# icyveins7/pydsproutines

Measured on AMD Instinct MI355X. Metric: CAF Msamples/s (4k template x 256 freq bins), higher is better.
Workload: dtype f32

## Files before the change

### pydsproutines_amd/csrc/caf_fft_dev.h

```cpp
#pragma once
#ifndef __HIPCC_RTC__
#include <hip/hip_runtime.h>
#endif

namespace caf {

__device__ __forceinline__ float2 cadd(float2 a, float2 b) { return make_float2(a.x + b.x, a.y + b.y); }
__device__ __forceinline__ float2 csub(float2 a, float2 b) { return make_float2(a.x - b.x, a.y - b.y); }
__device__ __forceinline__ float2 cmul(float2 a, float2 b) {
    return make_float2(__builtin_fmaf(a.x, b.x, -(a.y * b.y)), __builtin_fmaf(a.x, b.y, a.y * b.x));
}
__device__ __forceinline__ float2 mulj(float2 a) { return make_float2(-a.y, a.x); }
__device__ __forceinline__ void idft4(float2& a0, float2& a1, float2& a2, float2& a3) {
    const float2 s02 = cadd(a0, a2), d02 = csub(a0, a2);
    const float2 s13 = cadd(a1, a3), d13 = mulj(csub(a1, a3));
    a0 = cadd(s02, s13);
    a1 = cadd(d02, d13);
    a2 = csub(s02, s13);
    a3 = csub(d02, d13);
}

__device__ __forceinline__ void idft16(float2 (&v)[16]) {
    constexpr float C1 = 0.92387953251128674f;
    constexpr float S1 = 0.38268343236508977f;
    constexpr float R2 = 0.70710678118654752f;
#pragma unroll
    for (int m2 = 0; m2 < 4; ++m2) idft4(v[m2], v[4 + m2], v[8 + m2], v[12 + m2]);
    {
        const float2 w1 = make_float2(C1, S1), w3 = make_float2(S1, C1);
        v[4 * 1 + 1] = cmul(v[4 * 1 + 1], w1);
        v[4 * 2 + 1] = make_float2((v[4 * 2 + 1].x - v[4 * 2 + 1].y) * R2, (v[4 * 2 + 1].x + v[4 * 2 + 1].y) * R2);
        v[4 * 3 + 1] = cmul(v[4 * 3 + 1], w3);
        v[4 * 1 + 2] = make_float2((v[4 * 1 + 2].x - v[4 * 1 + 2].y) * R2, (v[4 * 1 + 2].x + v[4 * 1 + 2].y) * R2);
        v[4 * 2 + 2] = mulj(v[4 * 2 + 2]);
        v[4 * 3 + 2] = make_float2((-v[4 * 3 + 2].x - v[4 * 3 + 2].y) * R2, (v[4 * 3 + 2].x - v[4 * 3 + 2].y) * R2);
        v[4 * 1 + 3] = cmul(v[4 * 1 + 3], w3);
        v[4 * 2 + 3] = make_float2((-v[4 * 2 + 3].x - v[4 * 2 + 3].y) * R2, (v[4 * 2 + 3].x - v[4 * 2 + 3].y) * R2);
        v[4 * 3 + 3] = cmul(v[4 * 3 + 3], make_float2(-C1, -S1));
    }
#pragma unroll
    for (int n1 = 0; n1 < 4; ++n1) idft4(v[4 * n1 + 0], v[4 * n1 + 1], v[4 * n1 + 2], v[4 * n1 + 3]);
#pragma unroll
    for (int a = 0; a < 4; ++a)
#pragma unroll
        for (int b = a + 1; b < 4; ++b) {
            const float2 t = v[4 * a + b];
            v[4 * a + b] = v[4 * b + a];
            v[4 * b + a] = t;
        }
}

__device__ __forceinline__ void idft2(float2& a0, float2& a1) {
    const float2 s = cadd(a0, a1), d = csub(a0, a1);
    a0 = s;
    a1 = d;
}
__device__ __forceinline__ void idft8(float2 (&v)[8]) {
    constexpr float R2 = 0.70710678118654752f;
    float2 e0 = v[0], e1 = v[2], e2 = v[4], e3 = v[6];
    float2 o0 = v[1], o1 = v[3], o2 = v[5], o3 = v[7];
    idft4(e0, e1, e2, e3);
    idft4(o0, o1, o2, o3);
    o1 = make_float2((o1.x - o1.y) * R2, (o1.x + o1.y) * R2);
    o2 = mulj(o2);
    o3 = make_float2((-o3.x - o3.y) * R2, (o3.x - o3.y) * R2);
    v[0] = cadd(e0, o0);
    v[4] = csub(e0, o0);
    v[1] = cadd(e1, o1);
    v[5] = csub(e1, o1);
    v[2] = cadd(e2, o2);
    v[6] = csub(e2, o2);
    v[3] = cadd(e3, o3);
    v[7] = csub(e3, o3);
}

__device__ __forceinline__ void idft3(float2& x0, float2& x1, float2& x2) {
    constexpr float S = 0.86602540378443865f;
    const float2 t = cadd(x1, x2), d = csub(x1, x2);
    const float2 a = make_float2(x0.x - 0.5f * t.x, x0.y - 0.5f * t.y);
    const float2 b = make_float2(S * d.x, S * d.y);
    x0 = cadd(x0, t);
    x1 = make_float2(a.x - b.y, a.y + b.x);
    x2 = make_float2(a.x + b.y, a.y - b.x);
}
__device__ __forceinline__ void idft5(float2& x0, float2& x1, float2& x2, float2& x3, float2& x4) {
    constexpr float C1 = 0.30901699437494742f, C2 = -0.80901699437494742f;
    constexpr float S1 = 0.95105651629515357f, S2 = 0.58778525229247313f;
    const float2 t1 = cadd(x1, x4), t2 = cadd(x2, x3), t3 = csub(x1, x4), t4 = csub(x2, x3);
    const float2 a1 = make_float2(x0.x + C1 * t1.x + C2 * t2.x, x0.y + C1 * t1.y + C2 * t2.y);
    const float2 a2 = make_float2(x0.x + C2 * t1.x + C1 * t2.x, x0.y + C2 * t1.y + C1 * t2.y);
    const float2 b1 = make_float2(S1 * t3.x + S2 * t4.x, S1 * t3.y + S2 * t4.y);
    const float2 b2 = make_float2(S2 * t3.x - S1 * t4.x, S2 * t3.y - S1 * t4.y);
    x0 = make_float2(x0.x + t1.x + t2.x, x0.y + t1.y + t2.y);
    x1 = make_float2(a1.x - b1.y, a1.y + b1.x);
    x4 = make_float2(a1.x + b1.y, a1.y - b1.x);
    x2 = make_float2(a2.x - b2.y, a2.y + b2.x);
    x3 = make_float2(a2.x + b2.y, a2.y - b2.x);
}
__device__ __forceinline__ void idft10(float2 (&v)[10]) {
    float2 e0 = v[0], e1 = v[2], e2 = v[4], e3 = v[6], e4 = v[8];
    float2 o0 = v[1], o1 = v[3], o2 = v[5], o3 = v[7], o4 = v[9];
    idft5(e0, e1, e2, e3, e4);
    idft5(o0, o1, o2, o3, o4);
    o1 = cmul(o1, make_float2(0.80901699437494742f, 0.58778525229247313f));
    o2 = cmul(o2, make_float2(0.30901699437494742f, 0.95105651629515357f));
    o3 = cmul(o3, make_float2(-0.30901699437494742f, 0.95105651629515357f));
    o4 = cmul(o4, make_float2(-0.80901699437494742f, 0.58778525229247313f));
    v[0] = cadd(e0, o0), v[5] = csub(e0, o0);
    v[1] = cadd(e1, o1), v[6] = csub(e1, o1);
    v[2] = cadd(e2, o2), v[7] = csub(e2, o2);
    v[3] = cadd(e3, o3), v[8] = csub(e3, o3);
    v[4] = cadd(e4, o4), v[9] = csub(e4, o4);
}
__device__ __forceinline__ uint32_t fp_m2(uint32_t tid) {
    const uint32_t lane = tid & 63, wave = tid >> 6;
    const uint32_t b = (lane & 3) + 4 * (wave & 3), c = ((lane >> 2) & 3) + 4 * (wave >> 2), d = lane >> 4;
    return 64 * b + 4 * c + d;
}
__host__ __device__ __forceinline__ uint32_t fp_tid_of(uint32_t m2) {
    const uint32_t b = m2 >> 6, c = (m2 >> 2) & 15, d = m2 & 3;
    return (b & 3) | ((c & 3) << 2) | (d << 4) | ((b >> 2) << 6) | ((c >> 2) << 8);
}

}
```

### pydsproutines_amd/csrc/caf_fused.hip

```cpp
#include <algorithm>
#include <cstdlib>
#include <type_traits>

#include "caf_internal.h"
#include "caf_fft_dev.h"
#include "caf_wave.h"

namespace caf {

constexpr int FB = 16384;
constexpr int FP_P1 = 4384;
constexpr int FP_IM = 16 * FP_P1;
constexpr int F_LDS_BYTES = 2 * FP_IM;
constexpr int F_LDS_DATA = F_LDS_BYTES / 8;
__host__ __device__ constexpr int fp_row2(int n2) { return ((n2 >> 1) & 3) * 1088 + ((n2 & 1) + 2 * (n2 >> 3)) * 256; }
static_assert(fp_row2(15) + 256 <= FP_P1 && FP_P1 % 256 == 32, "planar image geometry");

#define CAF_AS1 __attribute__((address_space(1)))
#define CAF_AS4 __attribute__((address_space(4)))
typedef float v2f_t __attribute__((ext_vector_type(2)));
typedef float v4f_t __attribute__((ext_vector_type(4)));
typedef int v2i_t __attribute__((ext_vector_type(2)));
__device__ __forceinline__ float2 ld2(const float2* base, uint32_t elem) {
    const uint64_t u = *reinterpret_cast<const CAF_AS1 uint64_t*>((const CAF_AS1 char*)base + (elem << 3));
// ... 69 lines not shown
__device__ __forceinline__ float2 tw_ld(lds_tw_ptr b, int k) {
    const uint64_t u = b[k];
    float2 r;
    __builtin_memcpy(&r, &u, 8);
    return r;
}
__device__ __forceinline__ uint32_t fp_hbase(uint32_t m2, int32_t shift) {
    const uint32_t t = m2 - (uint32_t)shift;
    return (t & ~1023u) + fp_tid_of(t & 1023u);
}
__device__ __forceinline__ uint32_t fp_rd2(uint32_t tid) {
    const uint32_t lane = tid & 63, wave = tid >> 6;
    return wave * FP_P1 + (lane >> 4) * 1024 + (lane & 15) * 16;
}
__device__ __forceinline__ uint32_t fp_cd2(uint32_t tid) {
    const uint32_t lane = tid & 63;
    return 4 * ((lane & 3) + 4 * (lane >> 4)) + ((lane >> 2) & 3);
}
__device__ __forceinline__ uint32_t fp_rd3(uint32_t tid) {
    const uint32_t lane = tid & 63, wave = tid >> 6, n2 = lane >> 2;
    return wave * FP_P1 + ((n2 >> 1) & 3) * 1088 + ((n2 & 1) + 2 * (n2 >> 3)) * 256 + (lane & 3) * 16;
}
__device__ __forceinline__ uint32_t fp_rd4(uint32_t tid) {
    return (tid & 15) * FP_P1 + (tid >> 8) * 256 + ((tid >> 4) & 15) * 16;
}

template <typename Tp>
__device__ __forceinline__ Tp* uniform_ptr(Tp* p) {
    const uint64_t v = reinterpret_cast<uint64_t>(p);
    const uint32_t lo = __builtin_amdgcn_readfirstlane((uint32_t)v);
    const uint32_t hi = __builtin_amdgcn_readfirstlane((uint32_t)(v >> 32));
    return reinterpret_cast<Tp*>(((uint64_t)hi << 32) | lo);
}
__device__ __forceinline__ __amdgpu_buffer_rsrc_t buf_of(const void* base, uint32_t bytes) {
    return __builtin_amdgcn_make_buffer_rsrc(const_cast<void*>(base), 0, (int)bytes, 0x00020000);
}
constexpr int CAF_AUX_SC1 = 16;
constexpr int CAF_AUX_NT = 2;
template <int MODE>
__device__ __forceinline__ void tile_store(__amdgpu_buffer_rsrc_t r, uint32_t voff, uint32_t soff, float val) {
    __builtin_amdgcn_raw_buffer_store_b32(__builtin_bit_cast(int, val), r, (int)voff, (int)soff, MODE == 1 ? (CAF_AUX_SC1 | CAF_AUX_NT) : 0);
}

struct F1Direct {
    float* out0;
    float* out1;
    const float* inv_e;
    const float* tscale;
    int64_t num_shifts;
    int32_t step, blk_abs;
    PeakRec* partial;
    int64_t ppt, shift_start;
};
template <int FT, int MODE = 0, int NV4 = 4, bool PK = false>
__device__ __forceinline__ void fused_item(float2* __restrict__ s_d, const float2* __restrict__ s_tw2,
                                           const float2* __restrict__ s_tw3,
                                           const float2* __restrict__ xb,
                                           const float2* __restrict__ hc,
                                           const int32_t* __restrict__ shifts,
                                           const float2* __restrict__ tw1,
                                           int32_t table_mode, int32_t nfreq, int32_t nhyp, int blk, int h0, int h1,
                                           int32_t tiles_per_blk, float* __restrict__ vt,
                                           int32_t* __restrict__ imax = nullptr, const F1Direct* f1 = nullptr) {
    static_assert(FT == 1024, "one radix-16 butterfly per thread and pass: 1024 threads (wave w owns plane n1 = w)");
    constexpr int BPT = 1;
    const int tid = threadIdx.x;
    const lds_char* img = (const lds_char*)s_d;
    const uint32_t img0 = __builtin_amdgcn_readfirstlane((uint32_t)(uintptr_t)img);
    const uint32_t wave_u = __builtin_amdgcn_readfirstlane((uint32_t)tid >> 6);
    const uint32_t m0_x1 = img0 + wave_u * 256u, m0_w = img0 + wave_u * (uint32_t)FP_P1;
    const uint32_t m2 = fp_m2((uint32_t)tid);
    constexpr int nv4 = NV4;
    float bv[16];
    uint32_t bi[4];
    float ge[16];
    if (MODE == 2 || MODE == 5) {
#pragma unroll
        for (int o = 0; o < 16; ++o) bv[o] = -1.f;
#pragma unroll
        for (int o = 0; o < 4; ++o) bi[o] = 0u;
    }
    uint32_t f1_bytes = 0;
    int64_t f1_rel0 = 0;
    if (MODE >= 3) {
        f1_rel0 = (int64_t)f1->blk_abs * f1->step;
        int64_t nv = f1->num_shifts - f1_rel0;
        if (nv > f1->step) nv = f1->step;
        f1_bytes = (uint32_t)nv * 4u;
        const __amdgpu_buffer_rsrc_t rie = buf_of(uniform_ptr(f1->inv_e + f1_rel0), f1_bytes);
        const int n1 = tid & 15, n2 = (tid >> 4) & 15, q = tid >> 8;
#pragma unroll
        for (int i = 0; i < 4; ++i)
#pragma unroll
            for (int n4 = 0; n4 < 4; ++n4)
                ge[4 * i + n4] = __builtin_bit_cast(
                    float, __builtin_amdgcn_raw_buffer_load_b32(rie, (((n2 >> 2) + 4 * q) * 64 + n1 + 16 * (n2 & 3)) * 4,
                                                                (16 * i + 64 * n4) * 256, 0));
        if (MODE == 4) {
#pragma unroll
            for (int o = 0; o < 16; ++o) ge[o] = __builtin_sqrtf(ge[o]);
        }
    }

    uint32_t pk_d0 = 0, pk_nv = 0;
    if (PK) {
        const int n1 = tid & 15, n2 = (tid >> 4) & 15, q = tid >> 8;
        pk_d0 = (uint32_t)(((n2 >> 2) + 4 * q) * 64 + n1 + 16 * (n2 & 3));
        pk_nv = f1_bytes >> 2;
    }
    float2 w[BPT];
    const float2* xp = xb + (int64_t)blk * FB;
#pragma unroll
    for (int j = 0; j < BPT; ++j) w[j] = ld2(tw1, 1024u + m2);
    float* vt_blk = vt + (int64_t)blk * tiles_per_blk * nhyp * 64;
    const __amdgpu_buffer_rsrc_t rvt = buf_of(uniform_ptr(vt_blk), (uint32_t)tiles_per_blk * (uint32_t)nhyp * 256u);

    const float2* hrow_cur;
    uint32_t hb_cur;
    auto row_of = [&](int h) {
        if (table_mode) {
            hrow_cur = hc + (int64_t)h * FB;
            hb_cur = (uint32_t)tid;
        } else {
            const int t = h / nfreq;
            const int32_t sh = *((const CAF_AS4 int32_t*)shifts + (h - t * nfreq));
// ... 48 lines not shown
            float2 p = w[j];
            asm volatile("" : "+v"(p.x), "+v"(p.y));
            const float2 wj = p;
            v1[j][1] = cmul(v1[j][1], p);
#pragma unroll
            for (int n1 = 2; n1 < 16; ++n1) {
                p = cmul(p, wj);
                v1[j][n1] = cmul(v1[j][n1], p);
            }
        }
        __syncthreads();
        lds_rows16c<FP_P1>(m0_x1, v1[0]);
        __syncthreads();
        row_of(more ? h + 1 : h);
        constexpr int EH = MODE == 5 ? 2 : MODE >= 2 ? 5 : 0;
        float2 he[2 * EH + 1];
        constexpr int HP2 = 5;
        float2 hn[BPT][16];
        if (MODE < 2) {
#pragma unroll
            for (int a = 0; a < HP2; ++a) hn[0][a] = ld2(hrow_cur, ((1024u * a + hb_cur) & (FB - 1)) + lz);
        }
#pragma unroll
        for (int a = 0; a < EH; ++a) he[a] = ld2(hrow_cur, ((1024u * a + hb_cur) & (FB - 1)) + lz);
        {
            float2 v[16];
            const uint32_t rd2 = fp_rd2((uint32_t)(tid + lz)), rd2i = fp_im(rd2);
            const lds_tw_ptr t2 = tw_base(s_tw2, fp_cd2((uint32_t)(tid + lz)));
#pragma unroll
            for (int bh = 0; bh < 4; ++bh) lds_get4c(img, rd2 + 256u * bh, rd2i + 256u * bh, v[4 * bh], v[4 * bh + 1], v[4 * bh + 2], v[4 * bh + 3]);
            idft16(v);
#pragma unroll
            for (int n2 = 1; n2 < 16; ++n2) v[n2] = cmul(v[n2], tw_ld(t2, n2 * 64));
            lds_rows16c_x2(m0_w, v);
        }
#pragma unroll
        for (int a = 0; a < EH; ++a) pr[0][a] = cmul(xr[0][a], he[a]);
        __builtin_amdgcn_wave_barrier();
        if (MODE < 2) {
#pragma unroll
            for (int j = 0; j < BPT; ++j)
#pragma unroll
                for (int a = HP2; a < 16; ++a)
                    hn[j][a] = ld2(hrow_cur, (1024u * a + hb_cur) & (FB - 1));
        }
#pragma unroll
        for (int a = EH; a < 2 * EH; ++a) he[a] = ld2(hrow_cur, ((1024u * a + hb_cur) & (FB - 1)) + lz);
        {
            float2 v[16];
            const uint32_t rd3 = fp_rd3((uint32_t)(tid + lz)), rd3i = fp_im(rd3);
#pragma unroll
            for (int ch = 0; ch < 4; ++ch) lds_get4c(img, rd3 + 64u * ch, rd3i + 64u * ch, v[4 * ch], v[4 * ch + 1], v[4 * ch + 2], v[4 * ch + 3]);
            idft16(v);
            const lds_tw_ptr t3 = tw_base(s_tw3, (uint32_t)((tid & 3) + lz));
#pragma unroll
            for (int n3 = 1; n3 < 16; ++n3) v[n3] = cmul(v[n3], tw_ld(t3, n3 * 4));
            lds_rows16c<256>(m0_w, v);
        }
#pragma unroll
        for (int a = EH; a < 2 * EH; ++a) pr[0][a] = cmul(xr[0][a], he[a]);
        if (MODE >= 2) {
#pragma unroll
            for (int j = 0; j < BPT; ++j)
#pragma unroll
                for (int a = 2 * EH; a < 16; ++a)
                    hn[j][a] = ld2(hrow_cur, (1024u * a + hb_cur) & (FB - 1));
        }
        __syncthreads();
#pragma unroll
        for (int j = 0; j < BPT; ++j) {
            const int idx = tid + j * FT;
            const int n1 = idx & 15, n2 = (idx >> 4) & 15, q = idx >> 8;
            const uint32_t rd4 = fp_rd4((uint32_t)idx), rd4i = fp_im(rd4);
            __builtin_amdgcn_sched_barrier(0);
            float2 pf0, pf1, pf2, pf3;
            if (MODE < 2) {
                lds_get4c(img, rd4, rd4i, pf0, pf1, pf2, pf3);
                __builtin_amdgcn_sched_barrier(0);
#pragma unroll
                for (int a = 0; a < 16; ++a) pr[j][a] = cmul(xr[j][a], hn[j][a]);
                __builtin_amdgcn_sched_barrier(0);
            }
#pragma unroll
            for (int i = 0; i < 4; ++i) {
                uint32_t lzi = 0;
                asm volatile("" : "+v"(lzi));
                float2 a0, a1, a2, a3;
                if (MODE < 2 && i == 0)
                    a0 = pf0, a1 = pf1, a2 = pf2, a3 = pf3;
                else
                    lds_get4c(img, rd4 + 1024u * i + lzi, rd4i + 1024u * i + lzi, a0, a1, a2, a3);
                const float2 s02 = cadd(a0, a2), d02 = csub(a0, a2), s13 = cadd(a1, a3), d13 = mulj(csub(a1, a3));
#pragma unroll
                for (int n4 = 0; n4 < 4; ++n4) {
                    if (n4 >= nv4) continue;
                    const float2 yq = n4 == 0 ? cadd(s02, s13) : n4 == 1 ? cadd(d02, d13) : n4 == 2 ? csub(s02, s13) : csub(d02, d13);
                    const int tile_u = 16 * i + 64 * n4;
                    const int tile_t = (n2 >> 2) + 4 * q;
                    const uint32_t soff = (uint32_t)tile_u * (uint32_t)nhyp * 256u + hoff;
                    const uint32_t voff = ((uint32_t)tile_t * (uint32_t)nhyp * 64u + (uint32_t)(n1 + 16 * (n2 & 3))) << 2;
                    const float val = __builtin_fmaf(yq.x, yq.x, yq.y * yq.y);
                    if (MODE == 2) {
                        constexpr int o = 0;
                        (void)o;
                        const int oo = 4 * i + n4;
                        const bool up = val > bv[oo];
                        bv[oo] = up ? val : bv[oo];
                        const uint32_t sh8 = 8u * (uint32_t)(oo & 3);
                        const uint32_t repl = (bi[oo >> 2] & ~(0xffu << sh8)) | ((uint32_t)(h - h0) << sh8);
                        bi[oo >> 2] = up ? repl : bi[oo >> 2];
                    } else if (MODE == 5) {
                        const int oo = 4 * i + n4;
                        const float outv = val * (ge[oo] * f1_ts);
                        const bool up = outv > bv[oo];
                        bv[oo] = up ? outv : bv[oo];
                        const uint32_t sh8 = 8u * (uint32_t)(oo & 3);
                        const uint32_t repl = (bi[oo >> 2] & ~(0xffu << sh8)) | ((uint32_t)(h - h0) << sh8);
                        bi[oo >> 2] = up ? repl : bi[oo >> 2];
                        const uint32_t v3 = (uint32_t)(tile_t * 64 + n1 + 16 * (n2 & 3)) << 2, s3 = (uint32_t)tile_u * 256u;
                        __builtin_amdgcn_raw_buffer_store_b32(__builtin_bit_cast(int, outv), f1_r0, (int)v3, (int)s3, CAF_AUX_NT);
                    } else if (MODE == 4) {
                        const float gq = ge[4 * i + n4] * f1_ts;
                        const v2f_t ov = {yq.x * gq, yq.y * gq};
                        const uint32_t v3 = (uint32_t)(tile_t * 64 + n1 + 16 * (n2 & 3)) << 3, s3 = (uint32_t)tile_u * 512u;
                        __builtin_amdgcn_raw_buffer_store_b64(__builtin_bit_cast(v2i_t, ov), f1_r0, (int)v3, (int)s3, CAF_AUX_NT);
                    } else if (MODE == 3) {
                        const float outv = val * (ge[4 * i + n4] * f1_ts);
                        if (PK) {
                            const bool up = ((uint32_t)(pk_d0 + (16 * i + 64 * n4) * 64) < pk_nv) & (outv > pk_v[n4]);
                            pk_v[n4] = up ? outv : pk_v[n4];
                            pk_i[n4] = up ? (uint32_t)i : pk_i[n4];
                        }
                        const uint32_t v3 = (uint32_t)(tile_t * 64 + n1 + 16 * (n2 & 3)) << 2, s3 = (uint32_t)tile_u * 256u;
                        __builtin_amdgcn_raw_buffer_store_b32(__builtin_bit_cast(int, outv), f1_r0, (int)v3, (int)s3, CAF_AUX_NT);
                        if (f1->out1)
                            __builtin_amdgcn_raw_buffer_store_b32(__builtin_bit_cast(int, outv), f1_r1, (int)v3, (int)s3, CAF_AUX_NT);
                    } else {
                        tile_store<MODE>(rvt, voff, soff, val);
                    }
                }
                __builtin_amdgcn_sched_barrier(0);
            }
            if (MODE >= 2) {
#pragma unroll
                for (int a = 2 * EH; a < 16; ++a) pr[j][a] = cmul(xr[j][a], hn[j][a]);
            }
            __builtin_amdgcn_sched_barrier(0);
        }
        if (PK) {
            float bvv = pk_v[0];
            uint32_t bq = 0, bii = pk_i[0];
#pragma unroll
            for (int n4 = 1; n4 < NV4; ++n4) {
                const bool up = pk_v[n4] > bvv;
                bvv = up ? pk_v[n4] : bvv;
                bq = up ? (uint32_t)n4 : bq;
                bii = up ? pk_i[n4] : bii;
            }
            const uint32_t dloc = pk_d0 + (16u * bii + 64u * bq) * 64u;
            unsigned long long key = bvv < 0.f ? 0ull : (((unsigned long long)__float_as_uint(bvv) << 32) | (uint32_t)~dloc);
            key = wave_max(key);
            if ((tid & 63) == 0) {
                PeakRec r;
                r.v = key ? __uint_as_float((uint32_t)(key >> 32)) : -1.f;
                r.delay = key ? (int32_t)(f1->shift_start + f1_rel0 + (int64_t)(uint32_t)~(uint32_t)key) : 0x7fffffff;
                r.f = 0;
                f1->partial[(int64_t)h * f1->ppt + (int64_t)f1->blk_abs * 16 + (tid >> 6)] = r;
            }
        }
    }
    if (MODE == 2 || MODE == 5) {
        const int n1 = tid & 15, n2 = (tid >> 4) & 15, q = tid >> 8;
#pragma unroll
        for (int i = 0; i < 4; ++i)
#pragma unroll
            for (int n4 = 0; n4 < 4; ++n4) {
                const int tile = 16 * i + 64 * n4 + (n2 >> 2) + 4 * q;
                const int oo = 4 * i + n4;
                if (tile < tiles_per_blk) {
                    const uint32_t off = ((uint32_t)tile * 64u + (uint32_t)(n1 + 16 * (n2 & 3))) << 2;
                    gst1_wt(vt, off, bv[oo]);
                    __hip_atomic_store(reinterpret_cast<CAF_AS1 int32_t*>((CAF_AS1 char*)imax + off),
                                       (int32_t)(h0 + ((bi[oo >> 2] >> (8 * (oo & 3))) & 0xffu)), __ATOMIC_RELAXED,
                                       __HIP_MEMORY_SCOPE_AGENT);
                }
            }
    }
}

template <int N_> struct caf_ic { static constexpr int value = N_; };
template <int MODE, int NVH, bool FOLD, int R, bool PART = false>
__device__ __forceinline__ void fused_item2q(float2* __restrict__ s_d, const float2* __restrict__ s_tw2,
                                             const float2* __restrict__ s_tw3, const float2* __restrict__ xb,
                                             const float2* __restrict__ hc,
                                             const int32_t* __restrict__ shifts, const float2* __restrict__ tw1,
                                             int32_t table_mode, int32_t nfreq, int32_t nhyp, int blk, int h0, int h1,
                                             int32_t tiles_per_blk, float* __restrict__ vt, int32_t npart = 1,
                                             const F1Direct* __restrict__ f1 = nullptr) {
    static_assert(FOLD || R == 0, "the output residue exists in the folded form only");
    static_assert(MODE == 1 || MODE == 4, "|y|^2 tiles (write-through) or complex-QF rows");
    static_assert(!FOLD || NVH == 0, "folded form: only the lower half of each residue's transform holds valid delays");
    static_assert(!PART || FOLD, "partitioned templates ride on the folded form");
    constexpr int ROW = FOLD ? 4 * FB : 2 * FB;
    using pt_t = typename std::conditional<FOLD, float4, float2>::type;
    const int tid = threadIdx.x;
    const lds_char* img = (const lds_char*)s_d;
    const uint32_t img0 = __builtin_amdgcn_readfirstlane((uint32_t)(uintptr_t)img);
    const uint32_t wave_u = __builtin_amdgcn_readfirstlane((uint32_t)tid >> 6);
    const uint32_t m0_x1 = img0 + wave_u * 256u, m0_w = img0 + wave_u * (uint32_t)FP_P1;
    const uint32_t m2 = fp_m2((uint32_t)tid);
    const float2 w = ld2(tw1, 1024u + m2);
    float2 base0 = make_float2(1.f, 0.f);
    if (R) {
        float sn, cs;
        sincospif((float)m2 * (1.0f / 16384.0f), &sn, &cs);
        base0 = make_float2(cs, sn);
    }
    const float* xp = (const float*)(xb + (int64_t)blk * ROW);
    float* vt_blk = vt + (int64_t)blk * tiles_per_blk * nhyp * 64;
    const __amdgpu_buffer_rsrc_t rvt = buf_of(uniform_ptr(vt_blk), (uint32_t)tiles_per_blk * (uint32_t)nhyp * 256u);
    const int n1o = tid & 15, n2o = (tid >> 4) & 15, qo = tid >> 8;
    uint32_t f1_bytes = 0;
    int64_t f1_rel0 = 0;
    __amdgpu_buffer_rsrc_t rie = rvt, f1_r0 = rvt;
    float f1_ts = 0.f;
    if constexpr (MODE == 4) {
        f1_rel0 = (int64_t)f1->blk_abs * f1->step;
        int64_t nv = f1->num_shifts - f1_rel0;
        if (nv > f1->step) nv = f1->step;
        f1_bytes = (uint32_t)nv * 4u;
        rie = buf_of(uniform_ptr(f1->inv_e + f1_rel0), f1_bytes);
    }
    const float* hrow_o;
    uint32_t hb_o;
    const float* hrow_n;
    uint32_t hb_n;
    auto row_of = [&](int h, const float*& hrow, uint32_t& hb) {
        const int rows_per = PART ? npart : 1;
        if (table_mode) {
            hrow = (const float*)(hc + (int64_t)h * rows_per * ROW);
            hb = (uint32_t)tid;
        } else {
            const int t = h / nfreq;
// ... 285 lines not shown
    for (int64_t c = blockIdx.x; c < nchunks; c += gridDim.x)
        for (int j = threadIdx.x; j < 1024; j += 256) out[c * 1024 + j] = in[c * 1024 + fp_m2((uint32_t)j)];
}
void launch_butterfly_order(const float2* in, float2* out, int64_t nchunks, hipStream_t st) {
    hipLaunchKernelGGL(k_butterfly_order, dim3((unsigned)std::min<int64_t>(nchunks, 65535)), dim3(256), 0, st, in, out, nchunks);
}

template <bool BFLY>
__global__ __launch_bounds__(256) void k_parity_major(const float2* __restrict__ in, float2* __restrict__ out, int32_t half) {
    const float2* ir = in + (int64_t)blockIdx.y * 2 * half;
    float2* orow = out + (int64_t)blockIdx.y * 2 * half;
    for (int j = blockIdx.x * 256 + threadIdx.x; j < half; j += gridDim.x * 256) {
        const int m = BFLY ? (int)((j & ~1023) + fp_m2((uint32_t)j & 1023u)) : j;
        const float4 v = *reinterpret_cast<const float4*>(&ir[2 * m]);
        orow[j] = make_float2(v.x, v.y);
        orow[half + j] = make_float2(v.z, v.w);
    }
}
__global__ __launch_bounds__(256) void k_parity_pairs(const float2* __restrict__ in, float4* __restrict__ out, int32_t quarter) {
    const float2* ir = in + (int64_t)blockIdx.y * 4 * quarter;
    float4* orow = out + (int64_t)blockIdx.y * 2 * quarter;
    for (int j = blockIdx.x * 256 + threadIdx.x; j < quarter; j += gridDim.x * 256) {
        const int m = (int)((j & ~1023) + fp_m2((uint32_t)j & 1023u));
        const float4 lo = *reinterpret_cast<const float4*>(&ir[2 * m]), hi = *reinterpret_cast<const float4*>(&ir[2 * (m + quarter)]);
        orow[j] = make_float4(lo.x, lo.y, hi.x, hi.y);
        orow[quarter + j] = make_float4(lo.z, lo.w, hi.z, hi.w);
    }
}
void launch_parity_pairs(const float2* in, float2* out, int64_t rows, int32_t quarter, hipStream_t st) {
    for (int64_t r0 = 0; r0 < rows; r0 += 65535) {
        const int64_t nr = std::min<int64_t>(65535, rows - r0);
        hipLaunchKernelGGL(k_parity_pairs, dim3(16, (unsigned)nr), dim3(256), 0, st, in + r0 * 4 * quarter,
                           reinterpret_cast<float4*>(out + r0 * 4 * quarter), quarter);
    }
}
void launch_parity_major(const float2* in, float2* out, int64_t rows, int32_t half, hipStream_t st, bool butterfly) {
    for (int64_t r0 = 0; r0 < rows; r0 += 65535) {
        const int64_t nr = std::min<int64_t>(65535, rows - r0);
        if (butterfly)
            hipLaunchKernelGGL(k_parity_major<true>, dim3(16, (unsigned)nr), dim3(256), 0, st, in + r0 * 2 * half, out + r0 * 2 * half, half);
        else
            hipLaunchKernelGGL(k_parity_major<false>, dim3(16, (unsigned)nr), dim3(256), 0, st, in + r0 * 2 * half, out + r0 * 2 * half, half);
    }
}

template <int FT>
__global__ __launch_bounds__(FT) void k_fused_caf(const float2* __restrict__ xb, const float2* __restrict__ hc,
                                                  const int32_t* __restrict__ shifts, const float2* __restrict__ tw1,
                                                  const float2* __restrict__ tw23,
                                                  int32_t table_mode, int32_t nfreq, int32_t nhyp, int32_t hyp_per_wg,
                                                  int32_t nblk, int32_t tiles_per_blk, float* __restrict__ vt) {
    __shared__ __attribute__((aligned(16))) float2 s_d[F_LDS_DATA];
    __shared__ float2 s_tw2[16 * 64];
    __shared__ float2 s_tw3[16 * 4];
    const int tid = threadIdx.x;
    const int ngroups = (nhyp + hyp_per_wg - 1) / hyp_per_wg;
    const int lin = blockIdx.x;
    const int q = lin >> 3;
    const int blk = (q / ngroups) * 8 + (lin & 7);
    const int grp = q - (q / ngroups) * ngroups;
    if (blk >= nblk) return;
    const int h0 = grp * hyp_per_wg;
    const int h1 = min(h0 + hyp_per_wg, nhyp);

    for (int i = tid; i < 1024; i += FT) s_tw2[i] = tw23[i];
    if (tid < 64) s_tw3[tid] = tw23[1024 + tid];
    if (tiles_per_blk <= 192)
        fused_item<FT, 0, 3>(s_d, s_tw2, s_tw3, xb, hc, shifts, tw1, table_mode, nfreq, nhyp, blk, h0, h1, tiles_per_blk, vt);
    else
        fused_item<FT, 0, 4>(s_d, s_tw2, s_tw3, xb, hc, shifts, tw1, table_mode, nfreq, nhyp, blk, h0, h1, tiles_per_blk, vt);
}

template <int TR_F, bool NT_STORE>
__global__ __launch_bounds__(256) void k_transpose_norm_argmax(
    const float* __restrict__ vt, int32_t ntmpl, int32_t nfreq, const float* __restrict__ tscale,
    const float* __restrict__ inv_e, int64_t num_shifts, int64_t shift_start, int32_t step, int32_t blk0,
    int32_t tiles_per_blk, float* __restrict__ surface, float* __restrict__ row_max, int32_t* __restrict__ row_arg,
    PeakRec* __restrict__ partial, int64_t partial_per_tmpl) {
    __shared__ float s_tile[64][TR_F + 1];
    __shared__ float s_rowv[64];
    __shared__ int32_t s_rowi[64];
    const int z = blockIdx.z, t = blockIdx.y, tile = blockIdx.x;
    const int blk = blk0 + z;
    const int lane = threadIdx.x & 63, wave = threadIdx.x >> 6;
    const int sl0 = tile * 64;
    const int64_t rel0 = (int64_t)blk * step + sl0;
    int64_t nv = num_shifts - (int64_t)blk * step;
    if (nv > step) nv = step;
    const int64_t pidx = (int64_t)blk * tiles_per_blk + tile;
    if (sl0 >= nv) {
        if (threadIdx.x == 0 && partial) {
            PeakRec r;
            r.v = -1.f;
            r.delay = 0x7fffffff;
            r.f = 0;
            partial[(int64_t)t * partial_per_tmpl + pidx] = r;
        }
        return;
    }
    const int nrows = (int)min((int64_t)64, nv - sl0);
    const int nhyp = ntmpl * nfreq;
    const float* vin = vt + (((int64_t)z * tiles_per_blk + tile) * nhyp + (int64_t)t * nfreq) * 64;
    const int s4 = 4 * (threadIdx.x & 15);
    const float ts = tscale[t];
    float g[4];
#pragma unroll
    for (int k = 0; k < 4; ++k) g[k] = (s4 + k < nrows) ? inv_e[rel0 + s4 + k] * ts : -1.f;

    float bv[16];
    int32_t bi[16];
#pragma unroll
    for (int r = 0; r < 16; ++r) {
        bv[r] = -1.f;
        bi[r] = 0;
    }
    float4 q[TR_F / 16];
    auto load_chunk = [&](int f0) {
        const int nf = min(TR_F, nfreq - f0);
#pragma unroll
        for (int i = 0; i < TR_F / 16; ++i) {
            const int fl = i * 16 + (threadIdx.x >> 4);
            q[i] = (fl < nf) ? *reinterpret_cast<const float4*>(vin + (int64_t)(f0 + fl) * 64 + s4)
                             : make_float4(0.f, 0.f, 0.f, 0.f);
// ... 828 lines not shown
```

### pydsproutines_amd/csrc/caf_plan.hip

```cpp
#include <algorithm>
#include <cmath>
#include <complex>
#include <cstring>
#include <mutex>
#include <vector>

#include <unistd.h>

#include "caf_internal.h"

namespace caf {

static thread_local std::string g_last_error;
void set_error(const std::string& msg) { g_last_error = msg; }

}

using namespace caf;

static int env_int(const char* name, int dflt, bool* is_set = nullptr) {
    const char* e = getenv(name);
    if (is_set) *is_set = e != nullptr;
    return e ? atoi(e) : dflt;
}

constexpr uint32_t POISON_VT = 0x7149F2CAu;

namespace {
struct AuxSet {
    int dev;
    hipStream_t s;
    hipEvent_t fork, join;
};
std::mutex g_aux_mu;
std::vector<AuxSet> g_aux_idle;

int aux_acquire(int dev, hipStream_t* s, hipEvent_t* fork, hipEvent_t* join) {
    {
        std::lock_guard<std::mutex> lk(g_aux_mu);
        for (size_t i = 0; i < g_aux_idle.size(); ++i)
            if (g_aux_idle[i].dev == dev) {
                *s = g_aux_idle[i].s;
                *fork = g_aux_idle[i].fork;
                *join = g_aux_idle[i].join;
                g_aux_idle.erase(g_aux_idle.begin() + (long)i);
                return CAF_OK;
            }
    }
    CAF_HIP_TRY(hipStreamCreateWithFlags(s, hipStreamNonBlocking));
    CAF_HIP_TRY(hipEventCreateWithFlags(fork, hipEventDisableTiming));
    CAF_HIP_TRY(hipEventCreateWithFlags(join, hipEventDisableTiming));
    return CAF_OK;
}

void aux_release(int dev, hipStream_t s, hipEvent_t fork, hipEvent_t join) {
    if (s && fork && join) {
        std::lock_guard<std::mutex> lk(g_aux_mu);
        if (g_aux_idle.size() < 16) {
            g_aux_idle.push_back(AuxSet{dev, s, fork, join});
            return;
        }
    }
// ... 78 lines not shown
        for (auto& r : recs) {
            (void)hipEventSynchronize(r.b);
            float ms = 0.f;
            if (hipEventElapsedTime(&ms, r.a, r.b) == hipSuccess) {
                acc_ms[r.stage] += ms;
                acc_n[r.stage] += 1;
            }
            pool.push_back(r.a);
            pool.push_back(r.b);
        }
        recs.clear();
    }
    template <typename Tp>
    int alloc(Tp** p, int64_t count) {
        const int64_t bytes = count * (int64_t)sizeof(Tp);
        const int rc = pool_alloc((void**)p, std::max<int64_t>(bytes, 16));
        if (rc) return rc;
        workspace_bytes += bytes;
        return CAF_OK;
    }
    void release() {
        drain();
        (void)hipDeviceSynchronize();
        for (auto e : pool) (void)hipEventDestroy(e);
        pool.clear();
        fft_plan_release(&fwd);
        fft_plan_release(&inv);
        aux_release(device, s_aux, ev_fork, ev_join);
        s_aux = nullptr;
        ev_fork = ev_join = nullptr;
        void* ptrs[] = {d_dir_pos, d_dir_w, d_hc,  d_shifts, d_tscale, d_gstart,  d_glen, d_tile_sums, d_prefix, d_inv_e,
                        d_xb,  d_pbuf,   d_partial, d_vt,     d_params, d_pq,     d_uconj, d_nu,    d_xb2};
        for (void* p : ptrs)
            if (p) (void)pool_free(p);
    }
};

static int fused_twiddles(int device, float2** tw1_out, float2** tw23_out) {
    static std::mutex mu;
    static std::vector<std::pair<float2*, float2*>> per_dev;
    std::lock_guard<std::mutex> lk(mu);
    if ((int)per_dev.size() <= device) per_dev.resize(device + 1, {nullptr, nullptr});
    if (!per_dev[device].first) {
        std::vector<std::complex<float>> tw1(16 * 1024), tw23(2 * (16 * 64 + 16 * 4));
        auto cis = [](double num, double den) {
            const double ph = 2.0 * M_PI * std::fmod(num, den) / den;
            return std::complex<float>((float)std::cos(ph), (float)std::sin(ph));
        };
        for (int n1 = 0; n1 < 16; ++n1)
            for (int m2 = 0; m2 < 1024; ++m2) tw1[n1 * 1024 + m2] = cis((double)n1 * m2, 16384.0);
        for (int n2 = 0; n2 < 16; ++n2)
            for (int c = 0; c < 64; ++c) tw23[n2 * 64 + c] = cis((double)n2 * c, 1024.0);
        for (int n3 = 0; n3 < 16; ++n3)
            for (int dd = 0; dd < 4; ++dd) tw23[1024 + n3 * 4 + dd] = cis((double)n3 * dd, 64.0);
        for (int n2 = 0; n2 < 16; ++n2)
            for (int c = 0; c < 64; ++c) tw23[1088 + n2 * 64 + c] = cis((double)n2 * (2 * c + 1), 2048.0);
        for (int n3 = 0; n3 < 16; ++n3)
            for (int dd = 0; dd < 4; ++dd) tw23[1088 + 1024 + n3 * 4 + dd] = cis((double)n3 * (2 * dd + 1), 128.0);
        float2 *a = nullptr, *b = nullptr;
        int rc = upload_table(tw1.data(), (int64_t)tw1.size() * 8, false, (void**)&a);
        if (rc) return rc;
        if ((rc = upload_table(tw23.data(), (int64_t)tw23.size() * 8, false, (void**)&b))) {
            (void)hipFree(a);
            return rc;
        }
        per_dev[device] = {a, b};
    }
    *tw1_out = per_dev[device].first;
    *tw23_out = per_dev[device].second;
    return CAF_OK;
}

static int ilog2_ceil(int64_t v) {
    int l = 0;
    while (((int64_t)1 << l) < v) ++l;
    return l;
}

namespace caf {
int plan_zoom_view(caf_plan p, PlanZoomView* v) {
    CAF_REQUIRE(p && v, "NULL plan");
    v->T = p->T;
    v->N = p->N;
    v->F = p->F;
    v->G = p->G;
    v->device = p->device;
    v->d_uconj = p->d_uconj;
    v->d_nu = p->d_nu;
    v->d_tscale = p->d_tscale;
    return CAF_OK;
}
}

extern "C" {

int32_t caf_last_error(char* buf, int32_t len) {
    if (!buf || len <= 0) return CAF_ERR_INVALID;
    std::strncpy(buf, g_last_error.c_str(), (size_t)len - 1);
    buf[len - 1] = 0;
    return CAF_OK;
}

int32_t caf_abi_version(void) { return (1 << 16) | 10; }

int32_t caf_device_count(int32_t* count) {
    CAF_REQUIRE(count, "count is NULL");
    int n = 0;
// ... 957 lines not shown
```

Before: 1259.

## Fold third-pass twiddles into pass-4 radix-4 butterflies as compile-time constants

For modes below 2, the per-element twiddle multiply after the third FFT pass is dropped. Those twiddles are instead applied inside the fourth-pass radix-4 butterfly using compile-time cos/sin constants, picked by a switch on the wave index. This removes the LDS twiddle table loads and the separate complex multiplies, and frees the s_tw3 shared buffer. The cost is four specialised code paths per wave group, which grows code size, and the host twiddle table now uses the same constexpr values so results stay consistent.

```diff
diff --git a/pydsproutines_amd/csrc/caf_fft_dev.h b/pydsproutines_amd/csrc/caf_fft_dev.h
--- a/pydsproutines_amd/csrc/caf_fft_dev.h
+++ b/pydsproutines_amd/csrc/caf_fft_dev.h
@@ -3,15 +3,19 @@
 #include <hip/hip_runtime.h>
 #endif
 
+#ifndef CAF_FFT_FN
+#define CAF_FFT_FN __device__ __forceinline__
+#endif
+
 namespace caf {
 
-__device__ __forceinline__ float2 cadd(float2 a, float2 b) { return make_float2(a.x + b.x, a.y + b.y); }
-__device__ __forceinline__ float2 csub(float2 a, float2 b) { return make_float2(a.x - b.x, a.y - b.y); }
-__device__ __forceinline__ float2 cmul(float2 a, float2 b) {
+CAF_FFT_FN float2 cadd(float2 a, float2 b) { return make_float2(a.x + b.x, a.y + b.y); }
+CAF_FFT_FN float2 csub(float2 a, float2 b) { return make_float2(a.x - b.x, a.y - b.y); }
+CAF_FFT_FN float2 cmul(float2 a, float2 b) {
     return make_float2(__builtin_fmaf(a.x, b.x, -(a.y * b.y)), __builtin_fmaf(a.x, b.y, a.y * b.x));
 }
-__device__ __forceinline__ float2 mulj(float2 a) { return make_float2(-a.y, a.x); }
-__device__ __forceinline__ void idft4(float2& a0, float2& a1, float2& a2, float2& a3) {
+CAF_FFT_FN float2 mulj(float2 a) { return make_float2(-a.y, a.x); }
+CAF_FFT_FN void idft4(float2& a0, float2& a1, float2& a2, float2& a3) {
     const float2 s02 = cadd(a0, a2), d02 = csub(a0, a2);
     const float2 s13 = cadd(a1, a3), d13 = mulj(csub(a1, a3));
     a0 = cadd(s02, s13);
@@ -112,6 +116,65 @@
     v[3] = cadd(e3, o3), v[8] = csub(e3, o3);
     v[4] = cadd(e4, o4), v[9] = csub(e4, o4);
 }
+#define CAF_HD __host__ __device__ __forceinline__
+template <int NV = 4>
+CAF_HD void idft4_tw(float2 a0, float2 a1, float2 a2, float2 a3, float2 t1, float2 t2, float2 t3, float2 (&y)[4]) {
+    static_assert(NV >= 1 && NV <= 4, "output quarters");
+    const float2 u1 = make_float2(__builtin_fmaf(a1.x, t1.x, -(a1.y * t1.y)), __builtin_fmaf(a1.x, t1.y, a1.y * t1.x));
+    const float2 u2 = make_float2(__builtin_fmaf(a2.x, t2.x, -(a2.y * t2.y)), __builtin_fmaf(a2.x, t2.y, a2.y * t2.x));
+    const float2 u3 = make_float2(__builtin_fmaf(a3.x, t3.x, -(a3.y * t3.y)), __builtin_fmaf(a3.x, t3.y, a3.y * t3.x));
+    const float2 s02 = make_float2(a0.x + u2.x, a0.y + u2.y), s13 = make_float2(u1.x + u3.x, u1.y + u3.y);
+    y[0] = make_float2(s02.x + s13.x, s02.y + s13.y);
+    if (NV > 1) {
+        const float2 d02 = make_float2(a0.x - u2.x, a0.y - u2.y), e13 = make_float2(u1.x - u3.x, u1.y - u3.y);
+        y[1] = make_float2(d02.x - e13.y, d02.y + e13.x);
+        if (NV > 2) y[2] = make_float2(s02.x - s13.x, s02.y - s13.y);
+        if (NV > 3) y[3] = make_float2(d02.x + e13.y, d02.y - e13.x);
+    }
+}
+constexpr float W64_QUARTER[17] = {1.f,
+                                   0.99518472667219688624f,
+                                   0.98078528040323044913f,
+                                   0.95694033573220886494f,
+                                   0.92387953251128675613f,
+                                   0.88192126434835502971f,
+                                   0.83146961230254523708f,
+                                   0.77301045336273696081f,
+                                   0.70710678118654752440f,
+                                   0.63439328416364549822f,
+                                   0.55557023301960222474f,
+                                   0.47139673682599764856f,
+                                   0.38268343236508977173f,
+                                   0.29028467725446236764f,
+                                   0.19509032201612826785f,
+                                   0.09801714032956060199f,
+                                   6.123233995736766e-17f};
+constexpr int W64_KMAX = 45;
+constexpr float w64_cos(int k) {
+    return k <= 16 ? W64_QUARTER[k] : k <= 32 ? -W64_QUARTER[32 - k] : -W64_QUARTER[k - 32];
+}
+constexpr float w64_sin(int k) {
+    return k == 0 ? 0.f : k <= 16 ? W64_QUARTER[16 - k] : k < 32 ? W64_QUARTER[k - 16] : k == 32 ? 1.2246467991473532e-16f : -W64_QUARTER[48 - k];
+}
+template <int N3, int NV = 4>
+CAF_HD void idft4_w64(float2 a0, float2 a1, float2 a2, float2 a3, float2 (&y)[4]) {
+    static_assert(N3 >= 0 && N3 < 16 && 3 * N3 <= W64_KMAX, "third-pass output digit");
+    if (N3 == 0) {
+        const float2 s02 = make_float2(a0.x + a2.x, a0.y + a2.y), s13 = make_float2(a1.x + a3.x, a1.y + a3.y);
+        y[0] = make_float2(s02.x + s13.x, s02.y + s13.y);
+        if (NV > 1) {
+            const float2 d02 = make_float2(a0.x - a2.x, a0.y - a2.y), e13 = make_float2(a1.x - a3.x, a1.y - a3.y);
+            y[1] = make_float2(d02.x - e13.y, d02.y + e13.x);
+            if (NV > 2) y[2] = make_float2(s02.x - s13.x, s02.y - s13.y);
+            if (NV > 3) y[3] = make_float2(d02.x + e13.y, d02.y - e13.x);
+        }
+    } else {
+        constexpr float c1 = w64_cos(N3), s1 = w64_sin(N3), c2 = w64_cos(2 * N3), s2 = w64_sin(2 * N3), c3 = w64_cos(3 * N3),
+                        s3 = w64_sin(3 * N3);
+        idft4_tw<NV>(a0, a1, a2, a3, make_float2(c1, s1), make_float2(c2, s2), make_float2(c3, s3), y);
+    }
+}
+
 __device__ __forceinline__ uint32_t fp_m2(uint32_t tid) {
     const uint32_t lane = tid & 63, wave = tid >> 6;
     const uint32_t b = (lane & 3) + 4 * (wave & 3), c = ((lane >> 2) & 3) + 4 * (wave >> 2), d = lane >> 4;
diff --git a/pydsproutines_amd/csrc/caf_fused.hip b/pydsproutines_amd/csrc/caf_fused.hip
--- a/pydsproutines_amd/csrc/caf_fused.hip
+++ b/pydsproutines_amd/csrc/caf_fused.hip
@@ -145,6 +145,60 @@
     PeakRec* partial;
     int64_t ppt, shift_start;
 };
+#define CAF_PASS4_EMIT(i, n4, yq) \
+    do { \
+                const int tile_u = 16 * i + 64 * n4;                                             \
+                const int tile_t = (n2 >> 2) + 4 * q;                                                           \
+                const uint32_t soff = (uint32_t)tile_u * (uint32_t)nhyp * 256u + hoff;                  \
+                const uint32_t voff = ((uint32_t)tile_t * (uint32_t)nhyp * 64u + (uint32_t)(n1 + 16 * (n2 & 3))) << 2;               \
+                const float val = __builtin_fmaf(yq.x, yq.x, yq.y * yq.y);    \
+                if (MODE == 2) {                                                                                                     \
+                                                \
+                    constexpr int o = 0;                                                               \
+                    (void)o;                                                                                                         \
+                    const int oo = 4 * i + n4;                                                                                       \
+                    const bool up = val > bv[oo];                                                                                    \
+                    bv[oo] = up ? val : bv[oo];                                                                                      \
+                    const uint32_t sh8 = 8u * (uint32_t)(oo & 3);                                                                    \
+                    const uint32_t repl = (bi[oo >> 2] & ~(0xffu << sh8)) | ((uint32_t)(h - h0) << sh8);                             \
+                    bi[oo >> 2] = up ? repl : bi[oo >> 2];                                                                           \
+                } else if (MODE == 5) {                                                                                              \
+                                  \
+                                  \
+                                                                                         \
+                    const int oo = 4 * i + n4;                                                                                       \
+                    const float outv = val * (ge[oo] * f1_ts);                                                                       \
+                    const bool up = outv > bv[oo];                                                                                   \
+                    bv[oo] = up ? outv : bv[oo];                                                                                     \
+                    const uint32_t sh8 = 8u * (uint32_t)(oo & 3);                                                                    \
+                    const uint32_t repl = (bi[oo >> 2] & ~(0xffu << sh8)) | ((uint32_t)(h - h0) << sh8);                             \
+                    bi[oo >> 2] = up ? repl : bi[oo >> 2];                                                                           \
+                    const uint32_t v3 = (uint32_t)(tile_t * 64 + n1 + 16 * (n2 & 3)) << 2, s3 = (uint32_t)tile_u * 256u;             \
+                    __builtin_amdgcn_raw_buffer_store_b32(__builtin_bit_cast(int, outv), f1_r0, (int)v3, (int)s3, CAF_AUX_NT);       \
+                } else if (MODE == 4) {                                                                                              \
+                    const float gq = ge[4 * i + n4] * f1_ts;                                                                         \
+                    const v2f_t ov = {yq.x * gq, yq.y * gq};                                                                         \
+                    const uint32_t v3 = (uint32_t)(tile_t * 64 + n1 + 16 * (n2 & 3)) << 3, s3 = (uint32_t)tile_u * 512u;             \
+                    __builtin_amdgcn_raw_buffer_store_b64(__builtin_bit_cast(v2i_t, ov), f1_r0, (int)v3, (int)s3, CAF_AUX_NT);       \
+                } else if (MODE == 3) {                                                                                              \
+                               \
+                    const float outv = val * (ge[4 * i + n4] * f1_ts);                                                               \
+                    if (PK) {                                                                                                        \
+                                 \
+                               \
+                        const bool up = ((uint32_t)(pk_d0 + (16 * i + 64 * n4) * 64) < pk_nv) & (outv > pk_v[n4]);                   \
+                        pk_v[n4] = up ? outv : pk_v[n4];                                                                             \
+                        pk_i[n4] = up ? (uint32_t)i : pk_i[n4];                                                                      \
+                    }                                                                                                                \
+                    const uint32_t v3 = (uint32_t)(tile_t * 64 + n1 + 16 * (n2 & 3)) << 2, s3 = (uint32_t)tile_u * 256u;             \
+                    __builtin_amdgcn_raw_buffer_store_b32(__builtin_bit_cast(int, outv), f1_r0, (int)v3, (int)s3, CAF_AUX_NT);       \
+                    if (f1->out1)                                                                                                    \
+                        __builtin_amdgcn_raw_buffer_store_b32(__builtin_bit_cast(int, outv), f1_r1, (int)v3, (int)s3, CAF_AUX_NT);   \
+                } else {                                                                                                             \
+                    tile_store<MODE>(rvt, voff, soff, val);                  \
+                }                                                                                                                    \
+    } while (0)
+template <int N_> struct caf_ic { static constexpr int value = N_; };
 template <int FT, int MODE = 0, int NV4 = 4, bool PK = false>
 __device__ __forceinline__ void fused_item(float2* __restrict__ s_d, const float2* __restrict__ s_tw2,
                                            const float2* __restrict__ s_tw3,
@@ -164,6 +218,7 @@
     const uint32_t m0_x1 = img0 + wave_u * 256u, m0_w = img0 + wave_u * (uint32_t)FP_P1;
     const uint32_t m2 = fp_m2((uint32_t)tid);
     constexpr int nv4 = NV4;
+    constexpr bool MERGE34 = MODE < 2;
     float bv[16];
     uint32_t bi[4];
     float ge[16];
@@ -318,9 +373,11 @@
 #pragma unroll
             for (int ch = 0; ch < 4; ++ch) lds_get4c(img, rd3 + 64u * ch, rd3i + 64u * ch, v[4 * ch], v[4 * ch + 1], v[4 * ch + 2], v[4 * ch + 3]);
             idft16(v);
-            const lds_tw_ptr t3 = tw_base(s_tw3, (uint32_t)((tid & 3) + lz));
-#pragma unroll
-            for (int n3 = 1; n3 < 16; ++n3) v[n3] = cmul(v[n3], tw_ld(t3, n3 * 4));
+            if (!MERGE34) {
+                const lds_tw_ptr t3 = tw_base(s_tw3, (uint32_t)((tid & 3) + lz));
+#pragma unroll
+                for (int n3 = 1; n3 < 16; ++n3) v[n3] = cmul(v[n3], tw_ld(t3, n3 * 4));
+            }
             lds_rows16c<256>(m0_w, v);
         }
 #pragma unroll
@@ -345,67 +402,60 @@
                 __builtin_amdgcn_sched_barrier(0);
 #pragma unroll
                 for (int a = 0; a < 16; ++a) pr[j][a] = cmul(xr[j][a], hn[j][a]);
+#pragma unroll
+                for (int a = 0; a < 16; a += 4)
+                    asm volatile("" : "+v"(pr[j][a].x), "+v"(pr[j][a].y), "+v"(pr[j][a + 1].x), "+v"(pr[j][a + 1].y),
+                                      "+v"(pr[j][a + 2].x), "+v"(pr[j][a + 2].y), "+v"(pr[j][a + 3].x), "+v"(pr[j][a + 3].y));
                 __builtin_amdgcn_sched_barrier(0);
             }
-#pragma unroll
-            for (int i = 0; i < 4; ++i) {
-                uint32_t lzi = 0;
-                asm volatile("" : "+v"(lzi));
-                float2 a0, a1, a2, a3;
-                if (MODE < 2 && i == 0)
-                    a0 = pf0, a1 = pf1, a2 = pf2, a3 = pf3;
-                else
+            if constexpr (!MERGE34) {
+#pragma unroll
+                for (int i = 0; i < 4; ++i) {
+                    uint32_t lzi = 0;
+                    asm volatile("" : "+v"(lzi));
+                    float2 a0, a1, a2, a3;
                     lds_get4c(img, rd4 + 1024u * i + lzi, rd4i + 1024u * i + lzi, a0, a1, a2, a3);
-                const float2 s02 = cadd(a0, a2), d02 = csub(a0, a2), s13 = cadd(a1, a3), d13 = mulj(csub(a1, a3));
-#pragma unroll
-                for (int n4 = 0; n4 < 4; ++n4) {
-                    if (n4 >= nv4) continue;
-                    const float2 yq = n4 == 0 ? cadd(s02, s13) : n4 == 1 ? cadd(d02, d13) : n4 == 2 ? csub(s02, s13) : csub(d02, d13);
-                    const int tile_u = 16 * i + 64 * n4;
-                    const int tile_t = (n2 >> 2) + 4 * q;
-                    const uint32_t soff = (uint32_t)tile_u * (uint32_t)nhyp * 256u + hoff;
-                    const uint32_t voff = ((uint32_t)tile_t * (uint32_t)nhyp * 64u + (uint32_t)(n1 + 16 * (n2 & 3))) << 2;
-                    const float val = __builtin_fmaf(yq.x, yq.x, yq.y * yq.y);
-                    if (MODE == 2) {
-                        constexpr int o = 0;
-                        (void)o;
-                        const int oo = 4 * i + n4;
-                        const bool up = val > bv[oo];
-                        bv[oo] = up ? val : bv[oo];
-                        const uint32_t sh8 = 8u * (uint32_t)(oo & 3);
-                        const uint32_t repl = (bi[oo >> 2] & ~(0xffu << sh8)) | ((uint32_t)(h - h0) << sh8);
-                        bi[oo >> 2] = up ? repl : bi[oo >> 2];
-                    } else if (MODE == 5) {
-                        const int oo = 4 * i + n4;
-                        const float outv = val * (ge[oo] * f1_ts);
-                        const bool up = outv > bv[oo];
-                        bv[oo] = up ? outv : bv[oo];
-                        const uint32_t sh8 = 8u * (uint32_t)(oo & 3);
-                        const uint32_t repl = (bi[oo >> 2] & ~(0xffu << sh8)) | ((uint32_t)(h - h0) << sh8);
-                        bi[oo >> 2] = up ? repl : bi[oo >> 2];
-                        const uint32_t v3 = (uint32_t)(tile_t * 64 + n1 + 16 * (n2 & 3)) << 2, s3 = (uint32_t)tile_u * 256u;
-                        __builtin_amdgcn_raw_buffer_store_b32(__builtin_bit_cast(int, outv), f1_r0, (int)v3, (int)s3, CAF_AUX_NT);
-                    } else if (MODE == 4) {
-                        const float gq = ge[4 * i + n4] * f1_ts;
-                        const v2f_t ov = {yq.x * gq, yq.y * gq};
-                        const uint32_t v3 = (uint32_t)(tile_t * 64 + n1 + 16 * (n2 & 3)) << 3, s3 = (uint32_t)tile_u * 512u;
-                        __builtin_amdgcn_raw_buffer_store_b64(__builtin_bit_cast(v2i_t, ov), f1_r0, (int)v3, (int)s3, CAF_AUX_NT);
-                    } else if (MODE == 3) {
-                        const float outv = val * (ge[4 * i + n4] * f1_ts);
-                        if (PK) {
-                            const bool up = ((uint32_t)(pk_d0 + (16 * i + 64 * n4) * 64) < pk_nv) & (outv > pk_v[n4]);
-                            pk_v[n4] = up ? outv : pk_v[n4];
-                            pk_i[n4] = up ? (uint32_t)i : pk_i[n4];
-                        }
-                        const uint32_t v3 = (uint32_t)(tile_t * 64 + n1 + 16 * (n2 & 3)) << 2, s3 = (uint32_t)tile_u * 256u;
-                        __builtin_amdgcn_raw_buffer_store_b32(__builtin_bit_cast(int, outv), f1_r0, (int)v3, (int)s3, CAF_AUX_NT);
-                        if (f1->out1)
-                            __builtin_amdgcn_raw_buffer_store_b32(__builtin_bit_cast(int, outv), f1_r1, (int)v3, (int)s3, CAF_AUX_NT);
-                    } else {
-                        tile_store<MODE>(rvt, voff, soff, val);
+                    const float2 s02 = cadd(a0, a2), d02 = csub(a0, a2), s13 = cadd(a1, a3), d13 = mulj(csub(a1, a3));
+#pragma unroll
+                    for (int n4 = 0; n4 < 4; ++n4) {
+                        if (n4 >= nv4) continue;
+                        const float2 yq = n4 == 0 ? cadd(s02, s13) : n4 == 1 ? cadd(d02, d13) : n4 == 2 ? csub(s02, s13) : csub(d02, d13);
+                        CAF_PASS4_EMIT(i, n4, yq);
                     }
+                    __builtin_amdgcn_sched_barrier(0);
                 }
-                __builtin_amdgcn_sched_barrier(0);
+            } else {
+                auto sub = [&](auto qc, auto ic) __attribute__((always_inline)) {
+                    constexpr int i = decltype(ic)::value, N3 = decltype(qc)::value + 4 * i;
+                    uint32_t lzi = 0;
+                    asm volatile("" : "+v"(lzi));
+                    float2 a0, a1, a2, a3;
+                    if (i == 0)
+                        a0 = pf0, a1 = pf1, a2 = pf2, a3 = pf3;
+                    else
+                        lds_get4c(img, rd4 + 1024u * i + lzi, rd4i + 1024u * i + lzi, a0, a1, a2, a3);
+                    float2 y4[4];
+                    idft4_w64<N3, NV4>(a0, a1, a2, a3, y4);
+#pragma unroll
+                    for (int n4 = 0; n4 < 4; ++n4) {
+                        if (n4 >= nv4) continue;
+                        const float2 yq = y4[n4];
+                        CAF_PASS4_EMIT(i, n4, yq);
+                    }
+                    __builtin_amdgcn_sched_barrier(0);
+                };
+                auto steps = [&](auto qc) __attribute__((always_inline)) {
+                    sub(qc, caf_ic<0>{});
+                    sub(qc, caf_ic<1>{});
+                    sub(qc, caf_ic<2>{});
+                    sub(qc, caf_ic<3>{});
+                };
+                switch (wave_u >> 2) {
+                    case 0: steps(caf_ic<0>{}); break;
+                    case 1: steps(caf_ic<1>{}); break;
+                    case 2: steps(caf_ic<2>{}); break;
+                    default: steps(caf_ic<3>{}); break;
+                }
             }
             if (MODE >= 2) {
 #pragma unroll
@@ -454,7 +504,8 @@
     }
 }
 
-template <int N_> struct caf_ic { static constexpr int value = N_; };
+#undef CAF_PASS4_EMIT
+
 template <int MODE, int NVH, bool FOLD, int R, bool PART = false>
 __device__ __forceinline__ void fused_item2q(float2* __restrict__ s_d, const float2* __restrict__ s_tw2,
                                              const float2* __restrict__ s_tw3, const float2* __restrict__ xb,
@@ -846,7 +897,6 @@
                                                   int32_t nblk, int32_t tiles_per_blk, float* __restrict__ vt) {
     __shared__ __attribute__((aligned(16))) float2 s_d[F_LDS_DATA];
     __shared__ float2 s_tw2[16 * 64];
-    __shared__ float2 s_tw3[16 * 4];
     const int tid = threadIdx.x;
     const int ngroups = (nhyp + hyp_per_wg - 1) / hyp_per_wg;
     const int lin = blockIdx.x;
@@ -858,11 +908,10 @@
     const int h1 = min(h0 + hyp_per_wg, nhyp);
 
     for (int i = tid; i < 1024; i += FT) s_tw2[i] = tw23[i];
-    if (tid < 64) s_tw3[tid] = tw23[1024 + tid];
     if (tiles_per_blk <= 192)
-        fused_item<FT, 0, 3>(s_d, s_tw2, s_tw3, xb, hc, shifts, tw1, table_mode, nfreq, nhyp, blk, h0, h1, tiles_per_blk, vt);
+        fused_item<FT, 0, 3>(s_d, s_tw2, nullptr, xb, hc, shifts, tw1, table_mode, nfreq, nhyp, blk, h0, h1, tiles_per_blk, vt);
     else
-        fused_item<FT, 0, 4>(s_d, s_tw2, s_tw3, xb, hc, shifts, tw1, table_mode, nfreq, nhyp, blk, h0, h1, tiles_per_blk, vt);
+        fused_item<FT, 0, 4>(s_d, s_tw2, nullptr, xb, hc, shifts, tw1, table_mode, nfreq, nhyp, blk, h0, h1, tiles_per_blk, vt);
 }
 
 template <int TR_F, bool NT_STORE>
diff --git a/pydsproutines_amd/csrc/caf_plan.hip b/pydsproutines_amd/csrc/caf_plan.hip
--- a/pydsproutines_amd/csrc/caf_plan.hip
+++ b/pydsproutines_amd/csrc/caf_plan.hip
@@ -8,6 +8,7 @@
 #include <unistd.h>
 
 #include "caf_internal.h"
+#include "caf_fft_dev.h"
 
 namespace caf {
 
@@ -192,7 +193,8 @@
         for (int n2 = 0; n2 < 16; ++n2)
             for (int c = 0; c < 64; ++c) tw23[n2 * 64 + c] = cis((double)n2 * c, 1024.0);
         for (int n3 = 0; n3 < 16; ++n3)
-            for (int dd = 0; dd < 4; ++dd) tw23[1024 + n3 * 4 + dd] = cis((double)n3 * dd, 64.0);
+            for (int dd = 0; dd < 4; ++dd)
+                tw23[1024 + n3 * 4 + dd] = std::complex<float>(w64_cos(n3 * dd), w64_sin(n3 * dd));
         for (int n2 = 0; n2 < 16; ++n2)
             for (int c = 0; c < 64; ++c) tw23[1088 + n2 * 64 + c] = cis((double)n2 * (2 * c + 1), 2048.0);
         for (int n3 = 0; n3 < 16; ++n3)
```

Measured after the change: 1254. No clear change (-0.4%).
